# satoken/ractip

Hardware: AMD Instinct MI355X
Metric: sequence-pairs/sec (incl. bp+hp+ap DP; host strings in, thresholded matrices out) at n=500 (higher is better)
Workload: dtype f64; 1 GPU; synthetic random pairs n=500/500, std::mt19937(12345) stream (BASELINE config 3); scoring=CONTRAfold complementary (708 weights)

## Files before the change

### ractip_amd/csrc/compute.hip

```cpp
#include <hip/hip_runtime.h>

#include <algorithm>
#include <cmath>
#include <cstring>
#include <string>
#include <vector>

#include "ctx.h"
#include "kernels.h"

namespace rh::host {

template <class L, class... Args>
int run_graphed(rh_ctx* c, GraphSlot& g, hipStream_t stream, int k, L launcher, const Args&... args)
{
    const auto launch = [&] { int rc = RH_OK; ((rc = rc ? rc : launcher(c, args)), ...); return rc; };
    if (!c->use_graphs || c->time_cls >= 0) return launch();
    size_t key = 1469598103934665603ull + (sizeof(Args) + ...);
    const auto mix = [&](const void* p, size_t n) { for (size_t q = 0; q < n; q++) key = (key ^ ((const unsigned char*)p)[q]) * 0x100000001b3ull; };
    (mix(&args, sizeof(Args)), ...);
    int *launch_counter = &c->n_launch[k], *far_counter = &c->n_far[k];
    if (!g.exec || g.key != key) {
        if (g.exec) { HIP_TRY(c, hipGraphExecDestroy(g.exec)); g.exec = nullptr; }
        hipGraph_t graph = nullptr;
// ... 14 lines not shown
    }
    HIP_TRY(c, hipGraphLaunch(g.exec, stream));
    *launch_counter += g.launches;
    *far_counter += g.far;
    return RH_OK;
}

McLinArgs mc_lin_args(const rh_ctx* c, int phase, const McBatch& B, const LinSet* lin, bool routed)
{
    McLinArgs A;
    A.B = B; A.lin = lin; A.phase = phase;
    A.logz = c->d_mclogz.as<double>(); A.bad = c->d_bad.as<int>();
    A.plan = plan_mc_lin(c, phase, B.nmax);
    if (routed && (!c->small_list.empty() || c->n_short > 0)) {
        A.routed = 1;
        A.small_list = c->d_small_list.as<const int>(); A.n_small = (int)c->small_list.size();
        A.n_sweep = c->d_n_sweep.as<const int>(); A.nmax_sweep = c->nmax_sweep;
        A.n_short = c->d_n_short.as<const int>(); A.nmax_short = c->nmax_short; A.short_count = c->n_short;
        A.plan_sweep = plan_mc_lin(c, phase, A.nmax_sweep);
        A.plan_short = plan_mc_lin(c, phase, A.nmax_short);
    }
    A.pin = xcd_pin(B.ns);
    A.strip_xcd = c->strip_xcd;
    return A;
}

static McVlinArgs mc_vlin_args(const rh_ctx* c, int phase, bool co)
{
    McVlinArgs A;
    A.B = co ? c->co : c->mc; A.phase = phase; A.co = co;
    A.pin = xcd_pin(A.B.ns);
    A.plan = plan_mc_vlin(c, phase, co, A.B.nmax);
    A.d_vlin = c->d_vlin; A.h_vlin = c->h_vlin; A.hplen = c->h_hplen.data(); A.d_hplen = c->d_hplen.as<const double>();
    A.bad = co ? c->d_cobad.as<int>() : c->d_bad.as<int>();
    if (co) {
        const DxBatch& D = c->dx;
        if (A.B.seeded) { A.from = c->mc; A.pair_seq = c->d_pidx.as<const int>(); }
        A.hp = D.hp; A.hp_logz = D.logz; A.hp_stride = D.tab_stride; A.hp_ldd = D.ldd; A.n1max = D.n1max; A.n2max = D.n2max;
        A.cut_min = c->co_cut_min; A.cut_max = c->co_cut_max;
        A.window = c->co_window && c->co_cut_min >= 1 && (phase == 1 || A.B.seeded);
    } else {
        A.logz = c->d_mclogz.as<double>(); A.gaps = c->d_gaps.as<double>(); A.max_w = c->max_w;
        A.acc_wide = c->acc_wide && (size_t)VM_COUNT * A.B.tab_stride * sizeof(double) < ((size_t)1 << 32);
        A.acc_final_t = c->acc_final_t && c->max_w <= 15;
    }
    return A;
// ... 340 lines not shown
```

### ractip_amd/csrc/ctx.h

```cpp
#pragma once
#include <hip/hip_runtime.h>

#include <cassert>
#include <cstdint>
#include <cstring>
#include <string>
#include <type_traits>
#include <vector>

#include "../../include/ractip_hot.h"
#include "batch.h"
#include "score_model.h"
#include "lin_model.h"
#include "vienna_model.h"
#include "scale_order.h"

struct rh_ctx;

namespace rh::host {

struct DevBuf {
    void* p = nullptr;
    size_t cap = 0;
    DevBuf() = default;
// ... 44 lines not shown
    Far far = kFarNone;
    int far2_from = 0;
    int banded = 0;
    int repack2 = 0;
    const char* fine = "";
    const char* far_name = "";
};

static_assert(std::has_unique_object_representations_v<SweepPlan> && std::has_unique_object_representations_v<McBatch>);
static_assert(sizeof(DxLinBatch) == 4 * sizeof(void*) + 6 * sizeof(int) + 3 * sizeof(size_t) + 16 * sizeof(double), "no padding");

struct McLinArgs {
    McBatch B;
    const LinSet* lin;
    double* logz;
    int* bad;
    SweepPlan plan;
    const int* small_list;
    const int* n_sweep;
    const int* n_short;
    SweepPlan plan_sweep, plan_short;
    int routed, n_small, nmax_sweep, short_count, nmax_short;
    int phase, pin, strip_xcd;
    McLinArgs() { std::memset(this, 0, sizeof *this); }
};

struct McVlinArgs {
    McBatch B;
    McBatch from;
    const int* pair_seq;
    SweepPlan plan;
    const VLinModel* d_vlin;
    const VLinModel* h_vlin;
    const double* hplen;
    const double* d_hplen;
    int* bad;
    double* logz;
    double* gaps;
    double* hp;
    double* hp_logz;
    size_t hp_stride;
    int hp_ldd, n1max, n2max;
    int window, cut_min, cut_max;
    int max_w, acc_wide, acc_final_t;
    int phase, pin, co;
    McVlinArgs() { std::memset(this, 0, sizeof *this); }
// ... 70 lines not shown
    int dx_strip = 1;
    int dx_quad = 1;
    int dx_w = 4;
    int last_dx_path = 0;
    int far_mfma = 1;
    int lookahead = 2;
    int strip = 3;
    int far2 = -1;
    int strip_w = 8;
    int small_on = 0;
    std::vector<int> small_list;
    DevBuf d_small_list;
    DevBuf d_n_sweep;
    int nmax_sweep = 0;
    DevBuf d_n_short;
    int n_short = 0, nmax_short = 0;
    int strip_filt = 1;
    bool strip_filt_ok = false;
    int co_cut_min = 0, co_cut_max = 0;
    int co_window = 1;
    int acc_final_t = 1;
    int acc_wide = 1;
    int strip_xcd = 1;
    int far_pk = 1;
    int use_graphs = 1;
    GraphSlot g_in, g_out, g_dx;
    int mode = RH_MODE_AUTO;
    int duplex_mode = RH_MODE_INHERIT;
    int lin_w = 4;
    int lin_w_in = 4;
    int lin_bs = 16;
    int last_path = 0;
    bool last_went_log = false;
    SweepPlan plan[3];
    int max_w = 1;

    int np = 0, ns = 0;
    std::vector<int> pair_seq;
    std::vector<int> pair_seq_dev;
    bool indexed = false;
    bool has_mc = false, has_dx = false, computed = false;
    std::vector<int> n;
    McBatch mc = {};
    DxBatch dx = {};
    DevBuf d_seq;
    DevBuf d_n;
// ... 99 lines not shown
    assert(!"the plan names a kernel combination that has no row");
    return rows[0];
}
inline int xcd_pin(int ns) { return ns % 8 == 0 ? 1 : 0; }
inline dim3 seq_grid(int pin, int ns, int groups) { return pin ? dim3(ns, groups) : dim3(groups, ns); }
struct SweepPass {
    rh_ctx* c;
    const SweepPlan& P;
    const McBatch& B;
    hipStream_t st;
    int k;
    int far2_next = -1;
    int last_block() const { return P.BS > 0 ? (B.nmax - 1) / P.BS : 0; }
};
int launch_mc_log(rh_ctx* c, int pin, const McBatch& B, double* logz_out);
SweepPlan plan_mc_lin(const rh_ctx* c, int phase, int nmax);
int launch_mc_lin(rh_ctx* c, const McLinArgs& A);
void far_products(const rh_ctx* c, int phase, int nmax, bool mfma, SweepPlan* P);
const char* far_name(SweepPlan::Far far, int BS, int phase);
void far_inside_after(const SweepPass& S, int done);
void far_outside_begin(SweepPass& S, int top);
void far_outside_before(SweepPass& S, int d);
std::vector<double> strip_weights(const LinModel& L, bool* ok_out = nullptr);
int launch_mc_vienna(rh_ctx* c, int pin);
SweepPlan plan_mc_vlin(const rh_ctx* c, int phase, bool co, int nmax);
int launch_mc_vlin(rh_ctx* c, const McVlinArgs& A);
int launch_cofold(rh_ctx* c);
int select_vlin(rh_ctx* c, int model);
extern const double kVRungS[Ctx::kVRungs];
int launch_dx_log(rh_ctx* c, const DxBatch& D);
SweepPlan plan_dx_lin(const rh_ctx* c, int w);
SweepPlan plan_dx_vlin(bool sem20);
int launch_dx_lin(rh_ctx* c, const DxLinArgs& A);
int launch_dx_vlin(rh_ctx* c, const DxLinArgs& A);
int launch_dx_vlog(rh_ctx* c);
int retry_mc_lin_rungs(rh_ctx* c, int first_model, std::vector<int>* rest, int (&rescued_by)[Ctx::kRungs + 1]);
int recompute_mc_subset_log(rh_ctx* c, const std::vector<int>& F);
int retry_dx_lin_rungs(rh_ctx* c, std::vector<int>* rest);
int recompute_dx_subset_log(rh_ctx* c, const std::vector<int>& F);
int recompute_pairs_on_helper(rh_ctx* c, const std::vector<int>& P);
int compute(rh_ctx* c);
McLinArgs mc_lin_args(const rh_ctx* c, int phase, const McBatch& B, const LinSet* lin, bool routed);
DxLinArgs dx_lin_args(const rh_ctx* c);
int flagged(rh_ctx* c, const int* d_flags, int n, hipStream_t st, std::vector<int>* set);

}
// ... 3 lines not shown
```

### ractip_amd/csrc/kernels.h

```cpp
#pragma once
#include <hip/hip_runtime.h>

#include "../../include/ractip_hot.h"
#include "batch.h"
#include "score_model.h"
#include "lin_model.h"
#include "vienna_model.h"

namespace rh {
__global__ void mc_init(McBatch B);
__global__ void mc_inside_diag(McBatch B, const ScoreModel* __restrict__ M, int d, int pin);
__global__ void mc_outside_diag(McBatch B, const ScoreModel* __restrict__ M, int d, int pin);
__global__ void mc_unpaired(McBatch B);
__global__ void dx_sweep_diag(DxBatch B, const ScoreModel* __restrict__ M, int t);
__global__ void dx_logz(DxBatch B, const ScoreModel* __restrict__ M);
__global__ void dx_posterior(DxBatch B);
__global__ void dx_hp_clear_rest(DxBatch B);
__global__ void lin_init(McBatch B, const LinModel* __restrict__ L, int* __restrict__ bad);
template <int W, int BS, int MODE> __global__ void lin_inside_diag(McBatch B, const LinModel* __restrict__ L, int d, double lam_d, int pin);
template <int W, int BS> __global__ void lin_outside_diag(McBatch B, const LinModel* __restrict__ L, int d, int pin, int* __restrict__ bad);
template <int W, int BS> __global__ void lin_outside_pair(McBatch B, const LinModel* __restrict__ L, int d, int khi, int pin, int* __restrict__ bad);
template <int BS> __global__ void lin_far_inside(McBatch B, int D);
template <int BS> __global__ void lin_far_outside(McBatch B, int D);
__global__ void lin_far_inside_mfma(McBatch B, int D);
__global__ void lin_far_outside_mfma(McBatch B, int D);
template <int SWEEP> __global__ void lin_pack_tiles(McBatch B, int Dblk, int outside, int banded);
template <int KD, int W, int FILT> __global__ void lin_inside_strip(McBatch B, const LinModel* __restrict__ L, const double* __restrict__ wT, int d0, int f5_lo, double lam_d0, int pin);
template <int KD, int W, int FILT> __global__ void lin_outside_strip(McBatch B, const LinModel* __restrict__ L, const double* __restrict__ wT, int d0, int f5_hi, int f5_lo, int pin, int* __restrict__ bad);
__global__ void lin_f5i_tail(McBatch B, const LinModel* __restrict__ L, int jlo);
void launch_lin_small(const McBatch& B, const LinModel* L, const double* wpad, const int* list, int nlist, int* bad, hipStream_t stream);
__global__ void lin_f5o_head(McBatch B, const LinModel* __restrict__ L, int khi, int klo);
__global__ void lin_far_inside_pk(McBatch B, int D, int l2);
__global__ void lin_far_outside_pk(McBatch B, int D, int l2);
__global__ void lin_far2_inside(McBatch B, int D2, int l2);
__global__ void lin_far2_outside(McBatch B, int D2, int l2);
__global__ void lin_finish(McBatch B, const LinModel* __restrict__ L, double* __restrict__ logz, int* __restrict__ bad);
template <int W> __global__ void dxl_sweep(DxLinBatch B, const DxLinModel* __restrict__ L, int step, int groups);
__global__ void dxl_sweep4(DxLinBatch B, const DxLinModel* __restrict__ L, int step, int groups);
__global__ void dxl_strip8(DxLinBatch B, const DxLinModel* __restrict__ L, int step);
template <bool S20> __global__ void dxvl_sweep4(DxLinBatch B, const VLinModel* __restrict__ L, const VDxLin* __restrict__ D, int step);
template <bool S20> __global__ void dxvl_logz_part(DxLinBatch B, const VLinModel* __restrict__ L, const VDxLin* __restrict__ D, double* __restrict__ zpart,
                               int* __restrict__ cpart, int nchunk);
__global__ void dxvl_logz_final(DxLinBatch B, double s, const double* __restrict__ zpart, const int* __restrict__ cpart, int nchunk,
                                double* __restrict__ zbar, double* __restrict__ logz, int* __restrict__ bad);
constexpr int kLzThreads = 256;
size_t dxl_logz_lds_bytes(int lds);
__global__ void dxl_logz_part(DxLinBatch B, const DxLinModel* __restrict__ L, double* __restrict__ zpart, int* __restrict__ cpart, int nchunk);
__global__ void dxl_logz_final(DxLinBatch B, const DxLinModel* __restrict__ L, const double* __restrict__ zpart, const int* __restrict__ cpart, int nchunk,
                               double* __restrict__ zbar, double* __restrict__ logz, int* __restrict__ bad);
__global__ void dxl_posterior(DxLinBatch B, const double* __restrict__ zbar, int* __restrict__ bad);
__global__ void dxv_sweep_diag(DxBatch B, const ViennaDx* __restrict__ V, int t);
__global__ void dxv_logz(DxBatch B, const ViennaDx* __restrict__ V);
__global__ void dxv_posterior(DxBatch B);
__global__ void mcv_init(McBatch B);
// ... 49 lines not shown
```

### ractip_amd/csrc/launch_contrafold.hip

```cpp
#include <hip/hip_runtime.h>

#include <algorithm>
#include <cmath>
#include <cstring>
#include <string>
#include <vector>

#include "ctx.h"
#include "kernels.h"

__global__ void log_finish(rh::McBatch B, double* __restrict__ logz)
{
    const int sq = blockIdx.x * blockDim.x + threadIdx.x;
    if (sq < B.ns) logz[sq] = B.f5i[(size_t)sq * B.ld + B.n[sq]];
}

namespace rh::host {

int launch_mc_log(rh_ctx* c, int pin, const McBatch& B, double* logz_out)
{
    hipLaunchKernelGGL(mc_init, dim3((B.ns + 63) / 64), dim3(64), 0, c->s_mc, B);
    for (int d = 0; d <= B.nmax - 1; d++) {
        const int waves = std::max(B.nmax - 1 - d, 0) + 1;
        KLAUNCH(c, 0, mc_inside_diag, pin ? dim3(B.ns, (waves + 3) / 4) : dim3((waves + 3) / 4, B.ns), dim3(256), c->s_mc, B, c->d_model, d, pin);
// ... 128 lines not shown
        P.org = SweepPlan::kLookahead;
        P.fine = kInsideAhead[0].name;
    } else if (phase == 1 && mfma && (P.W == 4 || P.W == 8) && c->lookahead == 2) {
        P.org = SweepPlan::kPairs;
        P.fine = pair_kernels(P.W).out.name;
    }
    far_products(c, phase, nmax, mfma, &P);
    P.banded = strips;
    P.repack2 = phase == 1 && strips != (all_orgs && (c->strip & 1) && strips_ok);
    if (strips_on) P.fine = phase == 0 ? strip.in.name : strip.out.name;
    if (phase == 0 && P.org == SweepPlan::kPairs && !c->far_mfma) { P.fine = diag.in.name; P.far_name = far_name(SweepPlan::kFarLds, 16, 0); }
    return P;
}

static void inside_pairs(const SweepPass& S, const McLinArgs& A, int last)
{
    for (int d = 0; d <= last; d += 2) {
        const int groups = (std::max(S.B.nmax - 1 - d, 0) + 62) / 63 + 1;
        KLAUNCH(S.c, 0, (kInsidePair.kern), seq_grid(A.pin, S.B.ns, groups), dim3(256), S.st, S.B, A.lin->d, d, std::exp(-A.lin->h.s * d), A.pin);
        S.c->n_launch[0]++;
        far_inside_after(S, d + 2);
    }
}
static void inside_strips(const SweepPass& S, const McLinArgs& A)
{
    rh_ctx* c = S.c;
    const McBatch& B = S.B;
    constexpr int KD = 8, GS = 64 - (KD - 1);
    const auto strip = strip_kernels(S.P.W, S.P.filt).in.kern;
    inside_pairs(S, A, 30);
    int d0 = 32;
    for (; d0 <= B.nmax - 2; d0 += KD) {
        const int groups = (std::max(B.nmax - 1 - d0, 0) + GS - 1) / GS + 1;
        KLAUNCH(c, 0, strip, seq_grid(A.pin, B.ns, groups), dim3(64 * S.P.W), S.st, B, A.lin->d, A.lin->wT, d0, d0 == 32 ? 32 : d0 - KD + 2,
                std::exp(-A.lin->h.s * d0), (A.pin && A.strip_xcd) ? 2 : A.pin);
        c->n_launch[0]++;
        far_inside_after(S, d0 + KD);
    }
    hipLaunchKernelGGL(lin_f5i_tail, dim3(B.ns), dim3(256), 0, S.st, B, A.lin->d, d0 - KD + 2);
}
static void inside_diagonals(const SweepPass& S, const McLinArgs& A, bool ahead)
{
    const InsideDiagK full = diag_kernels(S.P.W, S.P.BS).in.kern;
    for (int d = 0; d <= S.B.nmax - 1; d++) {
        const int groups = (std::max(S.B.nmax - 1 - d, 0) + 63) / 64 + 1;
        const bool odd = ahead && (d & 1);
        KLAUNCH(S.c, 0, (!ahead ? full : kInsideAhead[odd].kern), seq_grid(A.pin, S.B.ns, groups), dim3(odd ? 64 : 64 * S.P.W), S.st, S.B, A.lin->d, d,
                std::exp(-A.lin->h.s * d), A.pin);
        S.c->n_launch[0]++;
        far_inside_after(S, d + 1);
    }
}

static void outside_strips(SweepPass& S, const McLinArgs& A)
{
    rh_ctx* c = S.c;
    const McBatch& B = S.B;
    constexpr int KD = 8, GS = 64 - (KD - 1);
    const auto strip = strip_kernels(S.P.W, S.P.filt).out.kern;
    const int d0_top = (B.nmax - 2) | (KD - 1);
    far_outside_begin(S, d0_top);
    hipLaunchKernelGGL(lin_f5o_head, dim3(B.ns), dim3(256), 0, S.st, B, A.lin->d, B.nmax - 1, d0_top - 5);
    for (int d0 = d0_top; d0 >= KD - 1; d0 -= KD) {
        far_outside_before(S, d0);
        const int groups = (std::max(B.nmax - 1 - (d0 - (KD - 1)), 0) + GS - 1) / GS + 1;
        KLAUNCH(c, 2, strip, seq_grid(A.pin, B.ns, groups), dim3(64 * S.P.W), S.st, B, A.lin->d, A.lin->wT, d0, d0 - 6, d0 - 13,
                (A.pin && A.strip_xcd) ? 2 : A.pin, A.bad);
        c->n_launch[1]++;
    }
}
static void outside_pairs(SweepPass& S, const McLinArgs& A)
{
    const auto pair = pair_kernels(S.P.W).out.kern;
    far_outside_begin(S, S.B.nmax - 2);
    for (int d = (S.B.nmax - 2) | 1; d >= 0; d -= 2) {
        for (int r = d; r >= d - 1 && r >= 0; r--) far_outside_before(S, r);
        const int ncol = S.B.nmax - 1 - d + 1;
        const int groups = std::max(1, (ncol - 1 + 62) / 63) + 1;
        KLAUNCH(S.c, 2, pair, seq_grid(A.pin, S.B.ns, groups), dim3(64 * S.P.W), S.st, S.B, A.lin->d, d, d, A.pin, A.bad);
        S.c->n_launch[1]++;
    }
}
static void outside_diagonals(SweepPass& S, const McLinArgs& A)
{
    const auto diag = diag_kernels(S.P.W, S.P.BS).out.kern;
    far_outside_begin(S, S.B.nmax - 2);
    for (int d = S.B.nmax - 2; d >= 0; d--) {
        far_outside_before(S, d);
        const int groups = (S.B.nmax - 1 - d + 63) / 64 + 1;
        KLAUNCH(S.c, 2, diag, seq_grid(A.pin, S.B.ns, groups), dim3(64 * S.P.W), S.st, S.B, A.lin->d, d, A.pin, A.bad);
// ... 85 lines not shown
```

### ractip_amd/csrc/mccaskill_strip.hip

```cpp
#include <hip/hip_runtime.h>

#include <type_traits>
#include <utility>

#include "batch.h"
#include "dev_util.h"
#include "lin_model.h"
#include "kernels.h"

namespace rh {

namespace {

template <int V> using IC = std::integral_constant<int, V>;
template <class F, int... Is> __device__ __forceinline__ void static_for_impl(F&& f, std::integer_sequence<int, Is...>) { (f(IC<Is>{}), ...); }
template <int N, class F> __device__ __forceinline__ void static_for(F&& f) { static_for_impl(f, std::make_integer_sequence<int, N>{}); }

}

#ifdef RH_STAMPS
__device__ unsigned long long g_stamps[16];
#define RH_STAMP(k) do { const unsigned long long t_ = __builtin_amdgcn_s_memtime(); st_acc_[k] += t_ - t_prev_; t_prev_ = t_; \
        if ((k) == 8 && threadIdx.x == 0) { for (int k_ = 0; k_ < 15; k_++) if (st_acc_[k_]) atomicAdd(&g_stamps[k_], st_acc_[k_]); atomicAdd(&g_stamps[15], 1ull); } } while (0)
#define RH_STAMP_BEGIN() unsigned long long st_acc_[15] = {}; unsigned long long t_prev_ = __builtin_amdgcn_s_memtime()
// ... 112 lines not shown
constexpr int kStripFiltOffD = 31 * 40;

template <int KD, int W>
struct InStripPlan {
    static constexpr int GS = 64 - (KD - 1);
    static constexpr int NM = 31;
    static constexpr int RD = NM + KD, CD = 72;
    static constexpr int RA = NM + KD, CA = 96;
    static constexpr int RE = 32, CE = 96;
    static constexpr int OFF_DUMMY = RD * CD + RA * CA + RE * CE;
    static constexpr int CS = 72;
    static constexpr int TS = 4;
    static constexpr bool SPLIT = W == 8 && KD == 8;
    static constexpr int PS = SPLIT ? 3 : 2;
    static constexpr int OFF_PART = KD * CD;
    static constexpr int OFF_S = OFF_PART + TS * KD * PS * 64;
    static constexpr int OFF_F1S = OFF_S + 5 * KD * CS;
    static constexpr int SZ = OFF_DUMMY + CA > OFF_F1S + (KD - 1) * 64 ? OFF_DUMMY + CA : OFF_F1S + (KD - 1) * 64;
};

constexpr int kWTS = 40;

template <int KD, int W, int FILT>
__global__ __launch_bounds__(64 * W, (W >= 8 ? 4 : 2)) void lin_inside_strip(McBatch B, const LinModel* __restrict__ L, const double* __restrict__ wT, int d0, int f5_lo,
                                                              double lam_d0, int pin)
{
    using P = InStripPlan<KD, W>;
    constexpr int GS = P::GS, NM = P::NM, CD = P::CD, CA = P::CA, CE = P::CE, CS = P::CS;
    constexpr int NSL = KD / W;
    constexpr int TS = P::TS, KH = KD * TS / W;
    static_assert(KD % W == 0 && KD <= 8 && W % TS == 0 && KD % (W / TS) == 0 && (NM + 1) % W == 0, "8 terms per end and term set, 32/W staged rows per wavefront and region");
    __shared__ double lds[P::SZ];
    __shared__ double red[W];
    constexpr bool FACT = FILT != 0 && W == 8 && KD == 8;
    __shared__ double fw[FACT ? 160 : 1];
    int sq = pin ? blockIdx.x : blockIdx.y, slot = pin ? blockIdx.y : blockIdx.x;
    if (pin == 2) {
        const unsigned lin = blockIdx.x + blockIdx.y * gridDim.x, t = lin >> 3;
        slot = (int)(t % gridDim.y);
        sq = (int)(t / gridDim.y) * 8 + (int)(lin & 7);
    }
    if (sq >= B.ns) return;
    const int n = B.n[sq];
    const int w = __builtin_amdgcn_readfirstlane(threadIdx.x >> 6), lane = threadIdx.x & 63;
    const int wt = w % TS, kb = (w / TS) * KH;
    const int ld = B.ld;
    const size_t ts = B.tab_stride;
    const uint8_t* __restrict__ s = B.seq + (size_t)sq * B.lds;
    double* __restrict__ tab = B.tab + (size_t)sq * B.seq_stride;
    double* __restrict__ f5i = B.f5i + (size_t)sq * ld;
    const int ncell0 = n - 1 - d0 > 0 ? n - 1 - d0 : 0;
    const int ngroup = (ncell0 + GS - 1) / GS;
    if (slot > ngroup) return;

    if (slot == ngroup) {
        const double* __restrict__ fca = tab + L_FCA * ts;
#pragma unroll 1
        for (int jj = f5_lo; jj <= d0 + 1; jj++) {
            if (jj < 1 || jj > n) continue;
            double acc = 0.0;
            if (threadIdx.x < 256)
                for (int k = threadIdx.x; k <= jj - 2; k += 256) acc = fma(f5i[k], fca[(size_t)(jj - 2 - k) * ld + (k + 1)], acc);
            acc = wsum(acc);
            if (lane == 0) red[w] = acc;
            __syncthreads();
            if (threadIdx.x == 0) f5i[jj] = f5i[jj - 1] * L->w_eu + (red[0] + red[1] + red[2] + red[3]) * L->w_ep2;
            __syncthreads();
        }
        return;
    }

#ifdef RH_STAGGER
    {
        const unsigned lin = blockIdx.x + blockIdx.y * gridDim.x;
        if (lin >= 256 && lin < 512) for (int q = 0; q < RH_STAGGER; q++) __builtin_amdgcn_s_sleep(127);
    }
#endif
    RH_STAMPI_BEGIN();
    RH_TRACE_ID(); RH_TRACE(1);
    const int i0 = 1 + slot * GS;
    const int i = i0 + lane;
    const int ic = i < ld ? i : ld - 1;
    double* const LDm = lds;
    double* const LA = lds + P::RD * CD;
    double* const LE = LA + P::RA * CA;
    const double* __restrict__ fm = tab + L_FM * ts;
    const double* __restrict__ fm1 = tab + L_FM1 * ts;
    const double* __restrict__ fcx = tab + L_FCX * ts;

    int s_j[NSL], s_jp1[NSL], s_jp2[NSL];
    int s_im1, s_i, s_ip1;
    int rb0, rb1, rb2, r0[NSL], r1[NSL], r2[NSL];
    {
// ... 380 lines not shown
        if constexpr (T >= 1 && T + 1 < KD)                                                         \
            static_for<KD>([&](auto KC) {                                                           \
                constexpr int K = decltype(KC)::value;                                              \
                if constexpr (K > T) { if (w == K % W) addrow(IC<(T >= 1 ? T - 1 : 0)>{}, KC); }    \
            });                                                                                     \
        if constexpr (T + 1 < KD) lds_barrier();                                                    \
    }
    RH_SLOT(0) RH_SLOT(1) RH_SLOT(2) RH_SLOT(3) RH_SLOT(4) RH_SLOT(5) RH_SLOT(6) RH_SLOT(7)
#undef RH_SLOT
    RH_STAMPI(7);
    lds_barrier();
    if (lane < GS) {
#pragma unroll 1
        for (int r = w; r < 5 * KD; r += W) {
            const int tb = r / KD, k = r - tb * KD, d = d0 + k;
            const int slot_of[5] = {L_FM, L_FM1, L_FCX, L_FC, L_FCA};
            if (i <= n - 1 - d) tab[slot_of[tb] * ts + (size_t)d * ld + i] = SFM[r * CS + lane];
        }
    }
    RH_STAMPI(8);
    RH_TRACE(4);
}

__global__ __launch_bounds__(256) void lin_f5i_tail(McBatch B, const LinModel* __restrict__ L, int jlo)
{
    __shared__ double red[4];
    const int sq = blockIdx.x;
    if (sq >= B.ns) return;
    const int n = B.n[sq], ld = B.ld;
    const int w = threadIdx.x >> 6, lane = threadIdx.x & 63;
    double* __restrict__ f5i = B.f5i + (size_t)sq * ld;
    const double* __restrict__ fca = B.tab + (size_t)sq * B.seq_stride + L_FCA * B.tab_stride;
#pragma unroll 1
    for (int jj = jlo < 1 ? 1 : jlo; jj <= n; jj++) {
        double acc = 0.0;
        for (int k = threadIdx.x; k <= jj - 2; k += 256) acc = fma(f5i[k], fca[(size_t)(jj - 2 - k) * ld + (k + 1)], acc);
        acc = wsum(acc);
        if (lane == 0) red[w] = acc;
        __syncthreads();
        if (threadIdx.x == 0) f5i[jj] = f5i[jj - 1] * L->w_eu + (red[0] + red[1] + red[2] + red[3]) * L->w_ep2;
        __syncthreads();
    }
}


template <int KD, int W>
struct OutStripPlan {
    static constexpr int GS = 64 - (KD - 1);
    static constexpr int NM = 31;
    static constexpr int TS = 4;
    static constexpr int RD = NM + KD, CD = 72;
    static constexpr int RA = NM + KD, CA = 96;
    static constexpr int RE = 32, CE = 96;
    static constexpr int OFF_DUMMY = RD * CD + RA * CA + RE * CE;
    static constexpr int SZ = OFF_DUMMY + CA + 320;
    static constexpr int PADL = 8, CS = 72;
    static constexpr int KEEP = (KD - 1) * CD;
    static constexpr int OFF_PART = KEEP;
    static constexpr int OFF_S = OFF_PART + TS * KD * 3 * 64;
    static_assert(OFF_S + 5 * KD * CS <= SZ, "overlay does not fit");
    static_assert(SZ * 8 <= 80 * 1024, "two workgroups per CU");
};

template <int W>
__device__ __forceinline__ void f5o_range(const double* __restrict__ fca_tab, double* __restrict__ f5o, const LinModel* __restrict__ L, int n, int ld,
                                          int khi, int klo, double* red)
{
    const int w = threadIdx.x >> 6, lane = threadIdx.x & 63;
#pragma unroll 1
    for (int k = khi; k >= klo && k >= 1; k--) {
        if (k > n - 1) continue;
        const double* __restrict__ fca = fca_tab + (k + 1);
        double acc = 0.0;
        if (threadIdx.x < 256)
            for (int jj = k + 2 + threadIdx.x; jj <= n; jj += 256) acc = fma(f5o[jj], fca[(size_t)(jj - 2 - k) * ld], acc);
        acc = wsum(acc);
        if (lane == 0) red[w] = acc;
        __syncthreads();
        if (threadIdx.x == 0) f5o[k] = f5o[k + 1] * L->w_eu + (red[0] + red[1] + red[2] + red[3]) * L->w_ep2;
        __syncthreads();
    }
}

__global__ __launch_bounds__(256) void lin_f5o_head(McBatch B, const LinModel* __restrict__ L, int khi, int klo)
{
    __shared__ double red[4];
    const int sq = blockIdx.x;
    if (sq >= B.ns) return;
    f5o_range<4>(B.tab + (size_t)sq * B.seq_stride + L_FCA * B.tab_stride, B.f5o + (size_t)sq * B.ld, L, B.n[sq], B.ld, khi, klo, red);
}

template <int KD, int W, int FILT>
__global__ __launch_bounds__(64 * W, (W >= 8 ? 4 : 2)) void lin_outside_strip(McBatch B, const LinModel* __restrict__ L, const double* __restrict__ wT, int d0, int f5_hi,
                                                                              int f5_lo, int pin, int* __restrict__ bad)
{
    using P = OutStripPlan<KD, W>;
    constexpr int GS = P::GS, NM = P::NM, CD = P::CD, CA = P::CA, CE = P::CE, CS = P::CS, PADL = P::PADL;
    constexpr int NSL = KD / W;
    constexpr int TS = P::TS, KH = KD * TS / W;
    static_assert(KD % W == 0 && KD <= 8 && W % TS == 0 && KD % (W / TS) == 0 && (NM + 1) % W == 0, "8 terms per end and term set, 32/W staged rows per wavefront and region");
    __shared__ double lds[P::SZ];
    __shared__ double red[W];
    constexpr bool FACT = FILT != 0 && W == 8 && KD == 8;
    __shared__ double fw[FACT ? 160 : 1];
    int sq = pin ? blockIdx.x : blockIdx.y, slot = pin ? blockIdx.y : blockIdx.x;
    if (pin == 2) {
        const unsigned lin = blockIdx.x + blockIdx.y * gridDim.x, t = lin >> 3;
        slot = (int)(t % gridDim.y);
        sq = (int)(t / gridDim.y) * 8 + (int)(lin & 7);
    }
    if (sq >= B.ns) return;
    const int n = B.n[sq];
    const int w = __builtin_amdgcn_readfirstlane(threadIdx.x >> 6), lane = threadIdx.x & 63;
    const int wt = w % TS, kb = (w / TS) * KH;
    const int ld = B.ld;
    const size_t ts = B.tab_stride;
    const uint8_t* __restrict__ s = B.seq + (size_t)sq * B.lds;
    double* __restrict__ tab = B.tab + (size_t)sq * B.seq_stride;
    const double* __restrict__ f5i = B.f5i + (size_t)sq * ld;
    double* __restrict__ f5o = B.f5o + (size_t)sq * ld;
    const int dlow = d0 - (KD - 1);
    const int ncell_max = n - 1 - dlow > 0 ? n - 1 - dlow : 0;
    const int ngroup = (ncell_max + GS - 1) / GS;
    if (slot > ngroup) return;
    if (slot == ngroup) {
        f5o_range<W>(tab + L_FCA * ts, f5o, L, n, ld, f5_hi, f5_lo, red);
        return;
    }

#ifdef RH_STAGGER
    {
        const unsigned lin = blockIdx.x + blockIdx.y * gridDim.x;
        if (lin >= 256 && lin < 512) for (int q = 0; q < RH_STAGGER; q++) __builtin_amdgcn_s_sleep(127);
    }
#endif
    RH_STAMPO_BEGIN();
    const int i0 = 1 + slot * GS - (KD - 1);
    const int i = i0 + lane;
    double* const LDm = lds;
    double* const LA = lds + P::RD * CD;
    double* const LE = LA + P::RA * CA;
    const double* __restrict__ fm = tab + L_FM * ts;
    const double* __restrict__ fm1 = tab + L_FM1 * ts;
    const double* __restrict__ fm2o = tab + L_FM2O * ts;
    const double* __restrict__ fcox = tab + L_FCOX * ts;

    int s_j[NSL], s_jp1[NSL], s_jp2[NSL];
    int s_im1, s_i, s_ip1;
    int rb0, rb1, rb2, r0[NSL], r1[NSL], r2[NSL];
    {
        const int top = B.lds - 1;
// ... 423 lines not shown
        double p = fco_s[sl] * p_fc[sl] * r_z;
        if (v && lane >= KD - 1 && (!(p == p) || p > 1e300)) { atomicOr(&bad[sq], 1); p = 0.0; }
        p = p > 1.0 ? 1.0 : (p < 0.0 ? 0.0 : p);
        if (!(p == p)) p = 0.0;
        PART[(K * 3) * 64 + lane] = p;
    }
    lds_barrier();
    if (lane >= KD - 1 && i >= 1) {
#pragma unroll 1
        for (int r = w; r < 5 * KD; r += W) {
            const int tb = r / KD, k = r - tb * KD, d = d0 - k;
            const int slot_of[5] = {L_FM2O, L_FMO, L_FM1O, L_FCO, L_FCOX};
            if (d >= 0 && i <= n - 1 - d) tab[slot_of[tb] * ts + (size_t)d * ld + i] = SFM2O[r * CS + PADL + lane];
        }
    }
    for (int t = threadIdx.x; t < 64 * KD; t += 64 * W) {
        const int c = t / KD, k = t - c * KD, ii = i0 + c, d = d0 - k;
        if (c >= KD - 1 && ii >= 1 && d >= 0 && ii <= n - 1 - d)
            B.bp[(size_t)sq * B.tri_stride + tri_off(n, ii) + (ii + d + 1)] = PART[(k * 3) * 64 + c];
    }
    RH_STAMPO(8);
}

template __global__ void lin_inside_strip<8, 4, 0>(McBatch, const LinModel*, const double*, int, int, double, int);
template __global__ void lin_inside_strip<8, 8, 0>(McBatch, const LinModel*, const double*, int, int, double, int);
template __global__ void lin_inside_strip<8, 8, 1>(McBatch, const LinModel*, const double*, int, int, double, int);
template __global__ void lin_outside_strip<8, 4, 0>(McBatch, const LinModel*, const double*, int, int, int, int, int*);
template __global__ void lin_outside_strip<8, 8, 0>(McBatch, const LinModel*, const double*, int, int, int, int, int*);
template __global__ void lin_outside_strip<8, 8, 1>(McBatch, const LinModel*, const double*, int, int, int, int, int*);

}
```

### ractip_amd/csrc/rh_api.hip

```cpp
#include <hip/hip_runtime.h>

#include <dlfcn.h>

#include <algorithm>
#include <cstdarg>
#include <cstdio>
#include <cstdlib>
#include <cstring>
#include <string>
#include <vector>

#include "ctx.h"
#include "kernels.h"

using namespace rh;
using namespace rh::host;

__global__ void collect_logz(const double* __restrict__ mc_logz, const int* __restrict__ idx, DxBatch D, double* __restrict__ out)
{
    const int p = blockIdx.x * blockDim.x + threadIdx.x;
    if (p >= D.np) return;
    out[3 * p + 0] = mc_logz[idx[2 * p]];
    out[3 * p + 1] = mc_logz[idx[2 * p + 1]];
    out[3 * p + 2] = D.logz[p];
// ... 73 lines not shown
}

enum EnvKind { ENV_INT, ENV_FLAG , ENV_NOT , ENV_4OR8 , ENV_DOUBLE };
struct EnvSwitch {
    const char* name;
    EnvKind kind;
    int Ctx::*field;
    double Ctx::*dfield = nullptr;
};
const EnvSwitch kEnvSwitches[] = {
    {"RH_LIN_W", ENV_INT, &Ctx::lin_w},        {"RH_LIN_W", ENV_INT, &Ctx::lin_w_in},
    {"RH_LIN_W_IN", ENV_INT, &Ctx::lin_w_in},
    {"RH_LIN_BS", ENV_INT, &Ctx::lin_bs},
    {"RH_NO_GRAPH", ENV_NOT, &Ctx::use_graphs},
    {"RH_FAR_MFMA", ENV_FLAG, &Ctx::far_mfma},
    {"RH_FAR_PK", ENV_FLAG, &Ctx::far_pk},
    {"RH_LOOKAHEAD", ENV_INT, &Ctx::lookahead},
    {"RH_STRIP", ENV_INT, &Ctx::strip},
    {"RH_STRIP_W", ENV_4OR8, &Ctx::strip_w},
    {"RH_STRIP_FILT", ENV_FLAG, &Ctx::strip_filt},
    {"RH_SMALL", ENV_FLAG, &Ctx::small_on},
    {"RH_FAR2", ENV_INT, &Ctx::far2},
    {"RH_STRIP_XCD", ENV_INT, &Ctx::strip_xcd},
    {"RH_ACC_WIDE", ENV_INT, &Ctx::acc_wide},
    {"RH_ACC_FINAL_T", ENV_INT, &Ctx::acc_final_t},
    {"RH_CO_WINDOW", ENV_INT, &Ctx::co_window},
    {"RH_SCALE_LADDER", ENV_INT, &Ctx::scale_ladder},
    {"RH_SCALE_MEMORY", ENV_INT, &Ctx::scale_memory},
    {"RH_PAIR_HELPER", ENV_INT, &Ctx::pair_helper},
    {"RH_CO_SEED", ENV_INT, &Ctx::co_seed},
    {"RH_DX_W", ENV_INT, &Ctx::dx_w},
    {"RH_DX_QUAD", ENV_FLAG, &Ctx::dx_quad},
    {"RH_DX_STRIP", ENV_INT, &Ctx::dx_strip},
    {"RH_VDX_S", ENV_DOUBLE, nullptr, &Ctx::vdx_s},
};

}

extern "C" {

static rh_ctx* create_ctx(int device, int model, const char* param_file, const char* defaults_file, int use_bl, int semantics);

rh_ctx* rh_create(int device, int model, const char* param_file) { return create_ctx(device, model, param_file, nullptr, 1, 0); }
rh_ctx* rh_create_vienna(int device, const char* defaults_file, int use_bl_param, const char* param_file, int semantics)
{
    return create_ctx(device, RH_MODEL_VIENNA_BL, param_file, defaults_file, use_bl_param, semantics);
// ... 469 lines not shown
```

Before: 11600 pairs/s.

## Move f5 inside/outside recurrences out of strip launches into single blocked LDS pass

Removes the extra per-strip workgroup that computed slices of the f5 inside and outside exterior-loop recurrences alongside each strip launch. Instead, a single dedicated kernel per sequence runs after the inside sweep, and another before the outside sweep, computing the whole f5 vector. Each kernel keeps f5 in LDS and batches 16 entries per global fetch pass, reducing global memory round trips. The trade-off is that this work becomes serial after or before the sweep rather than overlapped with the strips, and it adds LDS-size gating and more complex indexing.

Measured after the change: 12160 pairs/s, median of 6. +4.9%, better.

```diff
diff --git a/ractip_amd/csrc/compute.hip b/ractip_amd/csrc/compute.hip
--- a/ractip_amd/csrc/compute.hip
+++ b/ractip_amd/csrc/compute.hip
@@ -60,6 +60,8 @@
     }
     A.pin = xcd_pin(B.ns);
     A.strip_xcd = c->strip_xcd;
+    A.f5_jlo = 32;
+    A.f5_pass = c->f5_pass && f5_pass_lds(B.ld, 1) <= 64 * 1024;
     return A;
 }
 
diff --git a/ractip_amd/csrc/ctx.h b/ractip_amd/csrc/ctx.h
--- a/ractip_amd/csrc/ctx.h
+++ b/ractip_amd/csrc/ctx.h
@@ -90,6 +90,7 @@
     SweepPlan plan_sweep, plan_short;
     int routed, n_small, nmax_sweep, short_count, nmax_short;
     int phase, pin, strip_xcd;
+    int f5_pass, f5_jlo;
     McLinArgs() { std::memset(this, 0, sizeof *this); }
 };
 
@@ -206,6 +207,7 @@
     int acc_final_t = 1;
     int acc_wide = 1;
     int strip_xcd = 1;
+    int f5_pass = 1;
     int far_pk = 1;
     int use_graphs = 1;
     GraphSlot g_in, g_out, g_dx;
@@ -351,6 +353,7 @@
 void far_outside_begin(SweepPass& S, int top);
 void far_outside_before(SweepPass& S, int d);
 std::vector<double> strip_weights(const LinModel& L, bool* ok_out = nullptr);
+size_t f5_pass_lds(int ld, int phase);
 int launch_mc_vienna(rh_ctx* c, int pin);
 SweepPlan plan_mc_vlin(const rh_ctx* c, int phase, bool co, int nmax);
 int launch_mc_vlin(rh_ctx* c, const McVlinArgs& A);
diff --git a/ractip_amd/csrc/kernels.h b/ractip_amd/csrc/kernels.h
--- a/ractip_amd/csrc/kernels.h
+++ b/ractip_amd/csrc/kernels.h
@@ -25,11 +25,13 @@
 __global__ void lin_far_inside_mfma(McBatch B, int D);
 __global__ void lin_far_outside_mfma(McBatch B, int D);
 template <int SWEEP> __global__ void lin_pack_tiles(McBatch B, int Dblk, int outside, int banded);
-template <int KD, int W, int FILT> __global__ void lin_inside_strip(McBatch B, const LinModel* __restrict__ L, const double* __restrict__ wT, int d0, int f5_lo, double lam_d0, int pin);
-template <int KD, int W, int FILT> __global__ void lin_outside_strip(McBatch B, const LinModel* __restrict__ L, const double* __restrict__ wT, int d0, int f5_hi, int f5_lo, int pin, int* __restrict__ bad);
+template <int KD, int W, int FILT> __global__ void lin_inside_strip(McBatch B, const LinModel* __restrict__ L, const double* __restrict__ wT, int d0, double lam_d0, int pin);
+template <int KD, int W, int FILT> __global__ void lin_outside_strip(McBatch B, const LinModel* __restrict__ L, const double* __restrict__ wT, int d0, int pin, int* __restrict__ bad);
 __global__ void lin_f5i_tail(McBatch B, const LinModel* __restrict__ L, int jlo);
+__global__ void lin_f5i_pass(McBatch B, const LinModel* __restrict__ L, int jlo);
 void launch_lin_small(const McBatch& B, const LinModel* L, const double* wpad, const int* list, int nlist, int* bad, hipStream_t stream);
 __global__ void lin_f5o_head(McBatch B, const LinModel* __restrict__ L, int khi, int klo);
+__global__ void lin_f5o_pass(McBatch B, const LinModel* __restrict__ L);
 __global__ void lin_far_inside_pk(McBatch B, int D, int l2);
 __global__ void lin_far_outside_pk(McBatch B, int D, int l2);
 __global__ void lin_far2_inside(McBatch B, int D2, int l2);
diff --git a/ractip_amd/csrc/launch_contrafold.hip b/ractip_amd/csrc/launch_contrafold.hip
--- a/ractip_amd/csrc/launch_contrafold.hip
+++ b/ractip_amd/csrc/launch_contrafold.hip
@@ -174,6 +174,8 @@
         far_inside_after(S, d + 2);
     }
 }
+size_t f5_pass_lds(int ld, int phase) { return sizeof(double) * ((size_t)ld + 8 + (phase ? (size_t)((ld + 255) / 256) * 256 : 0)); }
+
 static void inside_strips(const SweepPass& S, const McLinArgs& A)
 {
     rh_ctx* c = S.c;
@@ -181,15 +183,15 @@
     constexpr int KD = 8, GS = 64 - (KD - 1);
     const auto strip = strip_kernels(S.P.W, S.P.filt).in.kern;
     inside_pairs(S, A, 30);
-    int d0 = 32;
-    for (; d0 <= B.nmax - 2; d0 += KD) {
-        const int groups = (std::max(B.nmax - 1 - d0, 0) + GS - 1) / GS + 1;
-        KLAUNCH(c, 0, strip, seq_grid(A.pin, B.ns, groups), dim3(64 * S.P.W), S.st, B, A.lin->d, A.lin->wT, d0, d0 == 32 ? 32 : d0 - KD + 2,
-                std::exp(-A.lin->h.s * d0), (A.pin && A.strip_xcd) ? 2 : A.pin);
+    for (int d0 = 32; d0 <= B.nmax - 2; d0 += KD) {
+        const int groups = (B.nmax - 1 - d0 + GS - 1) / GS;
+        KLAUNCH(c, 0, strip, seq_grid(A.pin, B.ns, groups), dim3(64 * S.P.W), S.st, B, A.lin->d, A.lin->wT, d0, std::exp(-A.lin->h.s * d0),
+                (A.pin && A.strip_xcd) ? 2 : A.pin);
         c->n_launch[0]++;
         far_inside_after(S, d0 + KD);
     }
-    hipLaunchKernelGGL(lin_f5i_tail, dim3(B.ns), dim3(256), 0, S.st, B, A.lin->d, d0 - KD + 2);
+    if (A.f5_pass) hipLaunchKernelGGL(lin_f5i_pass, dim3(B.ns), dim3(256), f5_pass_lds(B.ld, 0), S.st, B, A.lin->d, A.f5_jlo);
+    else hipLaunchKernelGGL(lin_f5i_tail, dim3(B.ns), dim3(256), 0, S.st, B, A.lin->d, A.f5_jlo);
 }
 static void inside_diagonals(const SweepPass& S, const McLinArgs& A, bool ahead)
 {
@@ -212,12 +214,12 @@
     const auto strip = strip_kernels(S.P.W, S.P.filt).out.kern;
     const int d0_top = (B.nmax - 2) | (KD - 1);
     far_outside_begin(S, d0_top);
-    hipLaunchKernelGGL(lin_f5o_head, dim3(B.ns), dim3(256), 0, S.st, B, A.lin->d, B.nmax - 1, d0_top - 5);
+    if (A.f5_pass) hipLaunchKernelGGL(lin_f5o_pass, dim3(B.ns), dim3(256), f5_pass_lds(B.ld, 1), S.st, B, A.lin->d);
+    else hipLaunchKernelGGL(lin_f5o_head, dim3(B.ns), dim3(256), 0, S.st, B, A.lin->d, B.nmax - 1, 1);
     for (int d0 = d0_top; d0 >= KD - 1; d0 -= KD) {
         far_outside_before(S, d0);
-        const int groups = (std::max(B.nmax - 1 - (d0 - (KD - 1)), 0) + GS - 1) / GS + 1;
-        KLAUNCH(c, 2, strip, seq_grid(A.pin, B.ns, groups), dim3(64 * S.P.W), S.st, B, A.lin->d, A.lin->wT, d0, d0 - 6, d0 - 13,
-                (A.pin && A.strip_xcd) ? 2 : A.pin, A.bad);
+        const int groups = (B.nmax - 1 - (d0 - (KD - 1)) + GS - 1) / GS;
+        KLAUNCH(c, 2, strip, seq_grid(A.pin, B.ns, groups), dim3(64 * S.P.W), S.st, B, A.lin->d, A.lin->wT, d0, (A.pin && A.strip_xcd) ? 2 : A.pin, A.bad);
         c->n_launch[1]++;
     }
 }
diff --git a/ractip_amd/csrc/mccaskill_strip.hip b/ractip_amd/csrc/mccaskill_strip.hip
--- a/ractip_amd/csrc/mccaskill_strip.hip
+++ b/ractip_amd/csrc/mccaskill_strip.hip
@@ -158,7 +158,7 @@
 constexpr int kWTS = 40;
 
 template <int KD, int W, int FILT>
-__global__ __launch_bounds__(64 * W, (W >= 8 ? 4 : 2)) void lin_inside_strip(McBatch B, const LinModel* __restrict__ L, const double* __restrict__ wT, int d0, int f5_lo,
+__global__ __launch_bounds__(64 * W, (W >= 8 ? 4 : 2)) void lin_inside_strip(McBatch B, const LinModel* __restrict__ L, const double* __restrict__ wT, int d0,
                                                               double lam_d0, int pin)
 {
     using P = InStripPlan<KD, W>;
@@ -167,7 +167,6 @@
     constexpr int TS = P::TS, KH = KD * TS / W;
     static_assert(KD % W == 0 && KD <= 8 && W % TS == 0 && KD % (W / TS) == 0 && (NM + 1) % W == 0, "8 terms per end and term set, 32/W staged rows per wavefront and region");
     __shared__ double lds[P::SZ];
-    __shared__ double red[W];
     constexpr bool FACT = FILT != 0 && W == 8 && KD == 8;
     __shared__ double fw[FACT ? 160 : 1];
     int sq = pin ? blockIdx.x : blockIdx.y, slot = pin ? blockIdx.y : blockIdx.x;
@@ -184,27 +183,9 @@
     const size_t ts = B.tab_stride;
     const uint8_t* __restrict__ s = B.seq + (size_t)sq * B.lds;
     double* __restrict__ tab = B.tab + (size_t)sq * B.seq_stride;
-    double* __restrict__ f5i = B.f5i + (size_t)sq * ld;
     const int ncell0 = n - 1 - d0 > 0 ? n - 1 - d0 : 0;
     const int ngroup = (ncell0 + GS - 1) / GS;
-    if (slot > ngroup) return;
-
-    if (slot == ngroup) {
-        const double* __restrict__ fca = tab + L_FCA * ts;
-#pragma unroll 1
-        for (int jj = f5_lo; jj <= d0 + 1; jj++) {
-            if (jj < 1 || jj > n) continue;
-            double acc = 0.0;
-            if (threadIdx.x < 256)
-                for (int k = threadIdx.x; k <= jj - 2; k += 256) acc = fma(f5i[k], fca[(size_t)(jj - 2 - k) * ld + (k + 1)], acc);
-            acc = wsum(acc);
-            if (lane == 0) red[w] = acc;
-            __syncthreads();
-            if (threadIdx.x == 0) f5i[jj] = f5i[jj - 1] * L->w_eu + (red[0] + red[1] + red[2] + red[3]) * L->w_ep2;
-            __syncthreads();
-        }
-        return;
-    }
+    if (slot >= ngroup) return;
 
 #ifdef RH_STAGGER
     {
@@ -631,6 +612,12 @@
     RH_TRACE(4);
 }
 
+__device__ __forceinline__ double f5_term(double f5, double fca, double acc) { return fma(f5, fca, acc); }
+__device__ __forceinline__ double f5_entry(double prev, double r0, double r1, double r2, double r3, double w_eu, double w_ep2)
+{
+    return fma(prev, w_eu, (r0 + r1 + r2 + r3) * w_ep2);
+}
+
 __global__ __launch_bounds__(256) void lin_f5i_tail(McBatch B, const LinModel* __restrict__ L, int jlo)
 {
     __shared__ double red[4];
@@ -643,15 +630,88 @@
 #pragma unroll 1
     for (int jj = jlo < 1 ? 1 : jlo; jj <= n; jj++) {
         double acc = 0.0;
-        for (int k = threadIdx.x; k <= jj - 2; k += 256) acc = fma(f5i[k], fca[(size_t)(jj - 2 - k) * ld + (k + 1)], acc);
+        for (int k = threadIdx.x; k <= jj - 2; k += 256) acc = f5_term(f5i[k], fca[(size_t)(jj - 2 - k) * ld + (k + 1)], acc);
         acc = wsum(acc);
         if (lane == 0) red[w] = acc;
         __syncthreads();
-        if (threadIdx.x == 0) f5i[jj] = f5i[jj - 1] * L->w_eu + (red[0] + red[1] + red[2] + red[3]) * L->w_ep2;
+        if (threadIdx.x == 0) f5i[jj] = f5_entry(f5i[jj - 1], red[0], red[1], red[2], red[3], L->w_eu, L->w_ep2);
         __syncthreads();
     }
 }
 
+constexpr int kF5Blk = 16;
+
+__global__ __launch_bounds__(256) void lin_f5i_pass(McBatch B, const LinModel* __restrict__ L, int jlo)
+{
+    extern __shared__ double f5_lds[];
+    const int sq = blockIdx.x;
+    if (sq >= B.ns) return;
+    const int n = B.n[sq], ld = B.ld;
+    if (n < jlo) return;
+    const int t = threadIdx.x, w = t >> 6, lane = t & 63;
+    double* const f5s = f5_lds;
+    double* const red = f5_lds + ld;
+    double* __restrict__ f5i = B.f5i + (size_t)sq * ld;
+    const double* __restrict__ fca = B.tab + (size_t)sq * B.seq_stride + L_FCA * B.tab_stride;
+    const double w_eu = L->w_eu, w_ep2 = L->w_ep2;
+    for (int k = t; k < jlo; k += 256) f5s[k] = f5i[k];
+    __syncthreads();
+    double prev = f5s[jlo - 1];
+#pragma unroll 1
+    for (int jj0 = jlo; jj0 <= n; jj0 += kF5Blk) {
+        const int ne = n - jj0 + 1 < kF5Blk ? n - jj0 + 1 : kF5Blk;
+        const int kmax = jj0 + ne - 3;
+        double acc[kF5Blk], opin[kF5Blk];
+#pragma unroll
+        for (int e = 0; e < kF5Blk; e++) { acc[e] = 0.0; opin[e] = 0.0; }
+        int kin = 0x7fffffff;
+        auto fetch = [&](int k, double (&op)[kF5Blk]) {
+            const int kc = k <= kmax ? k : kmax;
+            const double* __restrict__ col = fca + (kc + 1);
+#pragma unroll
+            for (int e = 0; e < kF5Blk; e++) {
+                const int row = jj0 + (e < ne ? e : 0) - 2 - kc;
+                op[e] = col[(size_t)(row > 0 ? row : 0) * ld];
+            }
+        };
+        auto take = [&](int k, const double (&op)[kF5Blk]) {
+            if (k > kmax) return;
+            if (k < jj0) {
+                const double f = f5s[k];
+#pragma unroll
+                for (int e = 0; e < kF5Blk; e++) acc[e] = (e < ne && (e > 0 || k <= jj0 - 2)) ? f5_term(f, op[e], acc[e]) : acc[e];
+            } else {
+                kin = k;
+#pragma unroll
+                for (int e = 2; e < kF5Blk; e++) opin[e] = op[e];
+            }
+        };
+#pragma unroll 1
+        for (int k = t; k <= kmax; k += 512) {
+            double opa[kF5Blk], opb[kF5Blk];
+            fetch(k, opa);
+            fetch(k + 256, opb);
+            take(k, opa);
+            take(k + 256, opb);
+        }
+#pragma unroll
+        for (int e = 0; e < kF5Blk; e++) {
+            if (e < ne) {
+                const int jj = jj0 + e;
+                double a = acc[e];
+                if (e >= 2 && kin <= jj - 2) a = f5_term(f5s[kin], opin[e], a);
+                a = wsum(a);
+                if (lane == 0) red[(e & 1) * 4 + w] = a;
+                lds_barrier();
+                const double* r = red + (e & 1) * 4;
+                prev = f5_entry(prev, r[0], r[1], r[2], r[3], w_eu, w_ep2);
+                if (t == 0) f5s[jj] = prev;
+            }
+        }
+        lds_barrier();
+        if (t < ne) f5i[jj0 + t] = f5s[jj0 + t];
+    }
+}
 
 template <int KD, int W>
 struct OutStripPlan {
@@ -671,37 +731,99 @@
     static_assert(SZ * 8 <= 80 * 1024, "two workgroups per CU");
 };
 
-template <int W>
-__device__ __forceinline__ void f5o_range(const double* __restrict__ fca_tab, double* __restrict__ f5o, const LinModel* __restrict__ L, int n, int ld,
-                                          int khi, int klo, double* red)
+__global__ __launch_bounds__(256) void lin_f5o_head(McBatch B, const LinModel* __restrict__ L, int khi, int klo)
 {
+    __shared__ double red[4];
+    const int sq = blockIdx.x;
+    if (sq >= B.ns) return;
+    const int n = B.n[sq], ld = B.ld;
     const int w = threadIdx.x >> 6, lane = threadIdx.x & 63;
+    const double* __restrict__ fca_tab = B.tab + (size_t)sq * B.seq_stride + L_FCA * B.tab_stride;
+    double* __restrict__ f5o = B.f5o + (size_t)sq * ld;
 #pragma unroll 1
     for (int k = khi; k >= klo && k >= 1; k--) {
         if (k > n - 1) continue;
         const double* __restrict__ fca = fca_tab + (k + 1);
         double acc = 0.0;
-        if (threadIdx.x < 256)
-            for (int jj = k + 2 + threadIdx.x; jj <= n; jj += 256) acc = fma(f5o[jj], fca[(size_t)(jj - 2 - k) * ld], acc);
+        for (int jj = k + 2 + threadIdx.x; jj <= n; jj += 256) acc = f5_term(f5o[jj], fca[(size_t)(jj - 2 - k) * ld], acc);
         acc = wsum(acc);
         if (lane == 0) red[w] = acc;
         __syncthreads();
-        if (threadIdx.x == 0) f5o[k] = f5o[k + 1] * L->w_eu + (red[0] + red[1] + red[2] + red[3]) * L->w_ep2;
+        if (threadIdx.x == 0) f5o[k] = f5_entry(f5o[k + 1], red[0], red[1], red[2], red[3], L->w_eu, L->w_ep2);
         __syncthreads();
     }
 }
 
-__global__ __launch_bounds__(256) void lin_f5o_head(McBatch B, const LinModel* __restrict__ L, int khi, int klo)
+__global__ __launch_bounds__(256) void lin_f5o_pass(McBatch B, const LinModel* __restrict__ L)
 {
-    __shared__ double red[4];
+    extern __shared__ double f5_lds[];
     const int sq = blockIdx.x;
     if (sq >= B.ns) return;
-    f5o_range<4>(B.tab + (size_t)sq * B.seq_stride + L_FCA * B.tab_stride, B.f5o + (size_t)sq * B.ld, L, B.n[sq], B.ld, khi, klo, red);
+    const int n = B.n[sq], ld = B.ld;
+    if (n < 2) return;
+    const int t = threadIdx.x, w = t >> 6, lane = t & 63;
+    double* const f5s = f5_lds;
+    double* const red = f5_lds + ld;
+    double* const park = red + 8;
+    const double* __restrict__ fca = B.tab + (size_t)sq * B.seq_stride + L_FCA * B.tab_stride;
+    double* __restrict__ f5o = B.f5o + (size_t)sq * ld;
+    const double w_eu = L->w_eu, w_ep2 = L->w_ep2;
+    double prev = f5o[n];
+    if (t == 0) f5s[n] = prev;
+    __syncthreads();
+#pragma unroll 1
+    for (int k0 = n - 1; k0 >= 1; k0 -= kF5Blk) {
+        const int ne = k0 < kF5Blk ? k0 : kF5Blk;
+        const int rmax = n - 2 - (k0 - ne + 1);
+        double acc[kF5Blk];
+#pragma unroll
+        for (int e = 0; e < kF5Blk; e++) acc[e] = 0.0;
+        auto fetch = [&](int r, double (&op)[kF5Blk]) {
+            const double* __restrict__ row = fca + (size_t)(r <= rmax ? r : 0) * ld;
+#pragma unroll
+            for (int e = 0; e < kF5Blk; e++) op[e] = row[k0 - (e < ne ? e : 0) + 1];
+        };
+        auto take = [&](int q, int r, const double (&op)[kF5Blk]) {
+            if (r > rmax) return;
+#pragma unroll
+            for (int e = 0; e < kF5Blk; e++) {
+                if (e >= 2 && t <= e - 2) park[(q * kF5Blk + e) * 16 + t] = op[e];
+                else if (e < ne && k0 - e + 2 + r <= n) acc[e] = f5_term(f5s[k0 - e + 2 + r], op[e], acc[e]);
+            }
+        };
+#pragma unroll 1
+        for (int q = 0; t + 256 * q <= rmax; q += 2) {
+            double opa[kF5Blk], opb[kF5Blk];
+            fetch(t + 256 * q, opa);
+            fetch(t + 256 * q + 256, opb);
+            take(q, t + 256 * q, opa);
+            take(q + 1, t + 256 * q + 256, opb);
+        }
+#pragma unroll
+        for (int e = 0; e < kF5Blk; e++) {
+            if (e < ne) {
+                const int k = k0 - e;
+                double a = acc[e];
+                if (e >= 2 && t <= e - 2) {
+                    a = 0.0;
+                    for (int q = 0; k + 2 + t + 256 * q <= n; q++) a = f5_term(f5s[k + 2 + t + 256 * q], park[(q * kF5Blk + e) * 16 + t], a);
+                }
+                a = wsum(a);
+                if (lane == 0) red[(e & 1) * 4 + w] = a;
+                lds_barrier();
+                const double* r = red + (e & 1) * 4;
+                prev = f5_entry(prev, r[0], r[1], r[2], r[3], w_eu, w_ep2);
+                if (t == 0) f5s[k] = prev;
+            }
+        }
+        lds_barrier();
+        if (t < ne) f5o[k0 - t] = f5s[k0 - t];
+    }
 }
 
 template <int KD, int W, int FILT>
-__global__ __launch_bounds__(64 * W, (W >= 8 ? 4 : 2)) void lin_outside_strip(McBatch B, const LinModel* __restrict__ L, const double* __restrict__ wT, int d0, int f5_hi,
-                                                                              int f5_lo, int pin, int* __restrict__ bad)
+__global__ __launch_bounds__(64 * W, (W >= 8 ? 4 : 2)) void lin_outside_strip(McBatch B, const LinModel* __restrict__ L, const double* __restrict__ wT, int d0,
+                                                                              int pin, int* __restrict__ bad)
 {
     using P = OutStripPlan<KD, W>;
     constexpr int GS = P::GS, NM = P::NM, CD = P::CD, CA = P::CA, CE = P::CE, CS = P::CS, PADL = P::PADL;
@@ -709,7 +831,6 @@
     constexpr int TS = P::TS, KH = KD * TS / W;
     static_assert(KD % W == 0 && KD <= 8 && W % TS == 0 && KD % (W / TS) == 0 && (NM + 1) % W == 0, "8 terms per end and term set, 32/W staged rows per wavefront and region");
     __shared__ double lds[P::SZ];
-    __shared__ double red[W];
     constexpr bool FACT = FILT != 0 && W == 8 && KD == 8;
     __shared__ double fw[FACT ? 160 : 1];
     int sq = pin ? blockIdx.x : blockIdx.y, slot = pin ? blockIdx.y : blockIdx.x;
@@ -731,11 +852,7 @@
     const int dlow = d0 - (KD - 1);
     const int ncell_max = n - 1 - dlow > 0 ? n - 1 - dlow : 0;
     const int ngroup = (ncell_max + GS - 1) / GS;
-    if (slot > ngroup) return;
-    if (slot == ngroup) {
-        f5o_range<W>(tab + L_FCA * ts, f5o, L, n, ld, f5_hi, f5_lo, red);
-        return;
-    }
+    if (slot >= ngroup) return;
 
 #ifdef RH_STAGGER
     {
@@ -1205,11 +1322,11 @@
     RH_STAMPO(8);
 }
 
-template __global__ void lin_inside_strip<8, 4, 0>(McBatch, const LinModel*, const double*, int, int, double, int);
-template __global__ void lin_inside_strip<8, 8, 0>(McBatch, const LinModel*, const double*, int, int, double, int);
-template __global__ void lin_inside_strip<8, 8, 1>(McBatch, const LinModel*, const double*, int, int, double, int);
-template __global__ void lin_outside_strip<8, 4, 0>(McBatch, const LinModel*, const double*, int, int, int, int, int*);
-template __global__ void lin_outside_strip<8, 8, 0>(McBatch, const LinModel*, const double*, int, int, int, int, int*);
-template __global__ void lin_outside_strip<8, 8, 1>(McBatch, const LinModel*, const double*, int, int, int, int, int*);
+template __global__ void lin_inside_strip<8, 4, 0>(McBatch, const LinModel*, const double*, int, double, int);
+template __global__ void lin_inside_strip<8, 8, 0>(McBatch, const LinModel*, const double*, int, double, int);
+template __global__ void lin_inside_strip<8, 8, 1>(McBatch, const LinModel*, const double*, int, double, int);
+template __global__ void lin_outside_strip<8, 4, 0>(McBatch, const LinModel*, const double*, int, int, int*);
+template __global__ void lin_outside_strip<8, 8, 0>(McBatch, const LinModel*, const double*, int, int, int*);
+template __global__ void lin_outside_strip<8, 8, 1>(McBatch, const LinModel*, const double*, int, int, int*);
 
 }
diff --git a/ractip_amd/csrc/rh_api.hip b/ractip_amd/csrc/rh_api.hip
--- a/ractip_amd/csrc/rh_api.hip
+++ b/ractip_amd/csrc/rh_api.hip
@@ -119,6 +119,7 @@
     {"RH_SMALL", ENV_FLAG, &Ctx::small_on},
     {"RH_FAR2", ENV_INT, &Ctx::far2},
     {"RH_STRIP_XCD", ENV_INT, &Ctx::strip_xcd},
+    {"RH_F5_PASS", ENV_FLAG, &Ctx::f5_pass},
     {"RH_ACC_WIDE", ENV_INT, &Ctx::acc_wide},
     {"RH_ACC_FINAL_T", ENV_INT, &Ctx::acc_final_t},
     {"RH_CO_WINDOW", ENV_INT, &Ctx::co_window},
```
